# maxjiang216/corintho-ai

Measured on AMD Instinct MI355X. Metric: self-play games/sec at 400 sims/move, higher is better.
Workload: dtype f32(f16x3)

## Files before the change

### corintho_ai_amd/csrc/nn_rescnn.hip

```cpp
#include <hip/hip_runtime.h>
#include <math.h>
#include <stdlib.h>
#include <string.h>

#include <vector>

#include "engine_defs.h"
#include <memory>

#include "host.h"
#include "lds_dma.h"
#include "nn_split.h"

#define RC_NB 4
#define RC_POS_PER_WG 16
#define RC_STEM_CHUNK 1024
#define RC_CONV_CHUNK 4096
#define RC_NUM_CONVS 9
#define RC_NUM_CHUNKS 81
#define RC_TRUNK_FLOATS (9 * RC_STEM_CHUNK + 72 * RC_CONV_CHUNK)

typedef float f32x4 __attribute__((ext_vector_type(4)));

struct RcParams {
  const float *in;
  const int32_t *d_rows;
  const float *wtrunk;
  const float *epi;
  const float *whead;
  const float *head_epi;
  const float *wpol;
  const float *bpol;
  const float *wv1;
  const float *bv1;
  const float *wv2;
  const float *bv2;
  float *eval;
  float *probs;
  CoNetIO io;
};

__device__ __forceinline__ size_t rc_in_row(const RcParams &P, int pos) { return (size_t)(P.io.in_idx ? P.io.in_idx[pos] : pos); }
__device__ __forceinline__ size_t rc_out_row(const RcParams &P, int pos) { return (size_t)(P.io.out_idx ? P.io.out_idx[pos] : pos); }

__device__ __forceinline__ const float *rc_chunk_ptr(const float *wtrunk, int ch) {
  return ch < 9 ? wtrunk + ch * RC_STEM_CHUNK : wtrunk + 9 * RC_STEM_CHUNK + (ch - 9) * RC_CONV_CHUNK;
}

__device__ __forceinline__ void rc_stage(const float *wtrunk, float *lds_buf, int ch, int wave, int lane) {
  const float *src = rc_chunk_ptr(wtrunk, ch);
  const int pieces = ch < 9 ? RC_STEM_CHUNK / 256 : RC_CONV_CHUNK / 256;
  for (int p = wave; p < pieces; p += 4) {
    __builtin_amdgcn_global_load_lds((const void __attribute__((address_space(1))) *)(src + p * 256 + lane * 4),
                                     (void __attribute__((address_space(3))) *)(lds_buf + p * 256), 16, 0, 0);
  }
}

template <int S>
__device__ __forceinline__ float rc_row_shift(float v) {
  if (S == 0) return v;
  constexpr int ctrl = S > 0 ? (0x100 + S) : (0x110 - S);
  return __int_as_float(__builtin_amdgcn_mov_dpp(__float_as_int(v), ctrl, 0xF, 0xF, true));
}

template <int TAP>
__device__ __forceinline__ float rc_tap(float v, bool okL, bool okR) {
  constexpr int dy = TAP / 3 - 1, dx = TAP % 3 - 1;
  float s = rc_row_shift<4 * dy + dx>(v);
  if (dx == -1) s = okL ? s : 0.0f;
  if (dx == 1) s = okR ? s : 0.0f;
  return s;
}

template <int CT, int TAP>
__device__ __forceinline__ void rc_conv_tap(f32x4 (&acc)[RC_NB][4], const float (&in)[RC_NB][4][4], const float *w, int lane,
                                            bool okL, bool okR) {
#pragma unroll
  for (int t = 0; t < CT; ++t) {
#pragma unroll
    for (int r = 0; r < 4; ++r) {
      const float *wp = w + ((t * 4 + r) * 4) * 64 + lane;
      float a[4];
#pragma unroll
      for (int to = 0; to < 4; ++to) a[to] = wp[to * 64];
#pragma unroll
      for (int nb = 0; nb < RC_NB; ++nb) {
        const float b = rc_tap<TAP>(in[nb][t][r], okL, okR);
#pragma unroll
        for (int to = 0; to < 4; ++to) acc[nb][to] = __builtin_amdgcn_mfma_f32_16x16x4f32(a[to], b, acc[nb][to], 0, 0, 0);
      }
    }
  }
}

template <int CT>
__device__ __forceinline__ void rc_conv3x3(f32x4 (&acc)[RC_NB][4], const float (&in)[RC_NB][4][4], int &ch,
                                           const float *wtrunk, float *lds_w, int wave, int lane, bool okL, bool okR) {
#pragma unroll
  for (int nb = 0; nb < RC_NB; ++nb)
#pragma unroll
    for (int to = 0; to < 4; ++to) acc[nb][to] = (f32x4){0.f, 0.f, 0.f, 0.f};
#define RC_TAP(T)                                                                         \
  {                                                                                       \
    asm volatile("s_waitcnt vmcnt(0)" ::: "memory");                                      \
    __syncthreads();                                                                      \
    if (ch + 1 < RC_NUM_CHUNKS) rc_stage(wtrunk, lds_w + ((ch + 1) & 1) * RC_CONV_CHUNK, ch + 1, wave, lane); \
    rc_conv_tap<CT, T>(acc, in, lds_w + (ch & 1) * RC_CONV_CHUNK, lane, okL, okR);        \
    ++ch;                                                                                 \
  }
  RC_TAP(0) RC_TAP(1) RC_TAP(2) RC_TAP(3) RC_TAP(4) RC_TAP(5) RC_TAP(6) RC_TAP(7) RC_TAP(8)
#undef RC_TAP
}

template <bool ADD_SKIP, bool RELU>
__device__ __forceinline__ void rc_epilogue(float (&out)[RC_NB][4][4], const f32x4 (&acc)[RC_NB][4],
                                            const float (&skip)[RC_NB][4][4], const float *epi, int q) {
#pragma unroll
  for (int to = 0; to < 4; ++to) {
    const float4 b4 = *reinterpret_cast<const float4 *>(epi + 16 * to + 4 * q);
    const float4 a4 = *reinterpret_cast<const float4 *>(epi + 64 + 16 * to + 4 * q);
    const float4 c4 = *reinterpret_cast<const float4 *>(epi + 128 + 16 * to + 4 * q);
    const float bb[4] = {b4.x, b4.y, b4.z, b4.w};
    const float aa[4] = {a4.x, a4.y, a4.z, a4.w};
    const float cc[4] = {c4.x, c4.y, c4.z, c4.w};
#pragma unroll
    for (int nb = 0; nb < RC_NB; ++nb)
#pragma unroll
      for (int r = 0; r < 4; ++r) {
        float v = acc[nb][to][r] + bb[r];
        v = aa[r] * v + cc[r];
        if (ADD_SKIP) v = skip[nb][to][r] + v;
        if (RELU) v = v > 0.0f ? v : 0.0f;
        out[nb][to][r] = v;
      }
  }
}

__device__ __forceinline__ void rc_dense_policy(const RcParams &P, const float *wpol, const float *feat16, int rows,
                                                int pos_base, int lane, int ncols = 16);
__device__ __forceinline__ void rc_dense_value(const RcParams &P, const float *wv1, const float *wv2, const float *feat16,
                                               int rows, int pos_base, int lane, int ncols = 16);

__device__ __forceinline__ void rc_heads(const RcParams &P, const float (&x)[RC_NB][4][4], float *feat_wg, int wave,
                                         int rows, int row0, int lane, int q, int c) {
  float *feat_w = feat_wg + wave * RC_NB * 96;
  f32x4 h1[RC_NB];
#pragma unroll
  for (int nb = 0; nb < RC_NB; ++nb) h1[nb] = (f32x4){0.f, 0.f, 0.f, 0.f};
#pragma unroll
  for (int t = 0; t < 4; ++t)
#pragma unroll
    for (int r = 0; r < 4; ++r) {
      const float a = P.whead[(t * 4 + r) * 64 + lane];
#pragma unroll
      for (int nb = 0; nb < RC_NB; ++nb) h1[nb] = __builtin_amdgcn_mfma_f32_16x16x4f32(a, x[nb][t][r], h1[nb], 0, 0, 0);
    }
  {
    const float4 b4 = *reinterpret_cast<const float4 *>(P.head_epi + 4 * q);
    const float4 a4 = *reinterpret_cast<const float4 *>(P.head_epi + 16 + 4 * q);
    const float4 c4 = *reinterpret_cast<const float4 *>(P.head_epi + 32 + 4 * q);
    const float bb[4] = {b4.x, b4.y, b4.z, b4.w};
    const float aa[4] = {a4.x, a4.y, a4.z, a4.w};
    const float cc[4] = {c4.x, c4.y, c4.z, c4.w};
#pragma unroll
    for (int nb = 0; nb < RC_NB; ++nb)
#pragma unroll
      for (int r = 0; r < 4; ++r) {
        float v = h1[nb][r] + bb[r];
        v = aa[r] * v + cc[r];
        v = v > 0.0f ? v : 0.0f;
        if (q == 0) feat_w[nb * 96 + c * 4 + r] = v;
        if (q == 1 && r < 2) feat_w[nb * 96 + 64 + c * 2 + r] = v;
      }
  }
  __syncthreads();
  if (wave == 0) rc_dense_policy(P, P.wpol, feat_wg, rows, row0, lane);
  if (wave == 1) rc_dense_value(P, P.wv1, P.wv2, feat_wg, rows, row0, lane);
}

__device__ __forceinline__ void rc_dense_policy(const RcParams &P, const float *wpol, const float *feat16, int rows,
                                                int pos_base, int lane, int ncols) {
  const int q = lane >> 4, c = lane & 15;
  const float *feat = feat16 + c * 96;
  f32x4 pl[6];
#pragma unroll
  for (int to = 0; to < 6; ++to) pl[to] = (f32x4){0.f, 0.f, 0.f, 0.f};
#pragma unroll
  for (int s = 0; s < 16; ++s) {
    const float b = feat[4 * s + q];
#pragma unroll
    for (int to = 0; to < 6; ++to)
      pl[to] = __builtin_amdgcn_mfma_f32_16x16x4f32(wpol[(s * 6 + to) * 64 + lane], b, pl[to], 0, 0, 0);
  }
  float lg[6][4];
  float m = -INFINITY;
#pragma unroll
  for (int to = 0; to < 6; ++to) {
    const float4 b4 = *reinterpret_cast<const float4 *>(P.bpol + 16 * to + 4 * q);
    const float bb[4] = {b4.x, b4.y, b4.z, b4.w};
#pragma unroll
    for (int r = 0; r < 4; ++r) {
      lg[to][r] = pl[to][r] + bb[r];
      m = lg[to][r] > m ? lg[to][r] : m;
    }
  }
  float o = __shfl_xor(m, 16, 64);
  m = o > m ? o : m;
  o = __shfl_xor(m, 32, 64);
  m = o > m ? o : m;
  float sum = 0.0f;
#pragma unroll
  for (int to = 0; to < 6; ++to)
#pragma unroll
    for (int r = 0; r < 4; ++r) {
      lg[to][r] = __builtin_amdgcn_exp2f((lg[to][r] - m) * 1.44269504088896340736f);
      sum += lg[to][r];
    }
  sum += __shfl_xor(sum, 16, 64);
  sum += __shfl_xor(sum, 32, 64);
  const float inv = 1.0f / sum;
  const int pos = pos_base + c;
  if (pos < rows && c < ncols) {
    const size_t orow = rc_out_row(P, pos);
#pragma unroll
    for (int to = 0; to < 6; ++to) {
      float4 p = make_float4(lg[to][0] * inv, lg[to][1] * inv, lg[to][2] * inv, lg[to][3] * inv);
      *reinterpret_cast<float4 *>(P.probs + orow * (size_t)P.io.probs_stride + 16 * to + 4 * q) = p;
    }
  }
}

__device__ __forceinline__ void rc_dense_value(const RcParams &P, const float *wv1, const float *wv2, const float *feat16,
                                               int rows, int pos_base, int lane, int ncols) {
  const int q = lane >> 4, c = lane & 15;
  const float *feat = feat16 + c * 96;
  f32x4 v1[4];
#pragma unroll
  for (int to = 0; to < 4; ++to) v1[to] = (f32x4){0.f, 0.f, 0.f, 0.f};
#pragma unroll
  for (int s = 0; s < 8; ++s) {
    const float b = feat[64 + 4 * s + q];
#pragma unroll
    for (int to = 0; to < 4; ++to)
      v1[to] = __builtin_amdgcn_mfma_f32_16x16x4f32(wv1[(s * 4 + to) * 64 + lane], b, v1[to], 0, 0, 0);
  }
  f32x4 v2 = (f32x4){0.f, 0.f, 0.f, 0.f};
#pragma unroll
  for (int t = 0; t < 4; ++t) {
    const float4 b4 = *reinterpret_cast<const float4 *>(P.bv1 + 16 * t + 4 * q);
    const float bb[4] = {b4.x, b4.y, b4.z, b4.w};
#pragma unroll
    for (int r = 0; r < 4; ++r) {
      float hv = v1[t][r] + bb[r];
      hv = hv > 0.0f ? hv : 0.0f;
      v2 = __builtin_amdgcn_mfma_f32_16x16x4f32(wv2[(t * 4 + r) * 64 + lane], hv, v2, 0, 0, 0);
    }
  }
  const int pos = pos_base + c;
  if (q == 0 && pos < rows && c < ncols) P.eval[rc_out_row(P, pos) * (size_t)P.io.eval_stride] = tanhf(v2[0] + P.bv2[0]);
}

#define CO_RC_F32_BLOCKS 2
__global__ __launch_bounds__(256, CO_RC_F32_BLOCKS) void co_k_rescnn_forward(RcParams P) {
  __shared__ __attribute__((aligned(16))) float lds_w[2 * RC_CONV_CHUNK];
  __shared__ float lds_feat[4][RC_NB][96];
  const int rows = *P.d_rows;
  const int row0 = blockIdx.x * RC_POS_PER_WG;
  if (row0 >= rows) return;
  const int tid = threadIdx.x;
  const int wave = tid >> 6, lane = tid & 63, q = lane >> 4, c = lane & 15;
  const bool okL = (c & 3) != 0, okR = (c & 3) != 3;
  rc_stage(P.wtrunk, lds_w, 0, wave, lane);

  float x[RC_NB][4][4];
#pragma unroll
  for (int nb = 0; nb < RC_NB; ++nb) {
    const int pos = row0 + wave * RC_NB + nb;
    float4 v = make_float4(0.f, 0.f, 0.f, 0.f);
    if (pos < rows) v = *reinterpret_cast<const float4 *>(P.in + rc_in_row(P, pos) * CO_STATE_STRIDE + (q == 0 ? 4 * c : 60 + 4 * q));
#pragma unroll
    for (int t = 0; t < 4; ++t)
#pragma unroll
      for (int r = 0; r < 4; ++r) x[nb][t][r] = 0.0f;
    x[nb][0][0] = v.x;
    x[nb][0][1] = v.y;
    x[nb][0][2] = v.z;
    x[nb][0][3] = v.w;
  }

  f32x4 acc[RC_NB][4];
  float y[RC_NB][4][4];
  int ch = 0;
  rc_conv3x3<1>(acc, x, ch, P.wtrunk, lds_w, wave, lane, okL, okR);
  rc_epilogue<false, true>(x, acc, x, P.epi, q);
  for (int b = 0; b < 4; ++b) {
    rc_conv3x3<4>(acc, x, ch, P.wtrunk, lds_w, wave, lane, okL, okR);
    rc_epilogue<false, true>(y, acc, x, P.epi + (size_t)(1 + 2 * b) * 192, q);
    rc_conv3x3<4>(acc, y, ch, P.wtrunk, lds_w, wave, lane, okL, okR);
    rc_epilogue<true, true>(x, acc, x, P.epi + (size_t)(2 + 2 * b) * 192, q);
  }

  rc_heads(P, x, &lds_feat[0][0][0], wave, rows, row0, lane, q, c);
}

#include "nn_rescnn_split.h"
#include "nn_rescnn_pix.h"

struct ResCnnNet : CoNet {
  std::vector<DevBuf<float>> bufs;
  RcParams P;
  size_t cap;

  float *upload(const std::vector<float> &h, rt_stream_t s) {
    bufs.emplace_back();
    bufs.back().upload(h.data(), h.size(), s);
    return bufs.back().p;
  }

  ResCnnNet(const float *w, size_t max_rows, rt_stream_t s) : cap(max_rows) {
    constexpr ResCnnLayout RL;
    std::vector<float> trunk(RC_TRUNK_FLOATS, 0.0f), epi((size_t)RC_NUM_CONVS * 192, 0.0f);
    size_t off = 0;
    for (int cv = 0; cv < RC_NUM_CONVS; ++cv) {
      const int cin = RL.cin(cv), ct = cv == 0 ? 1 : 4;
      const size_t chunk = cv == 0 ? RC_STEM_CHUNK : RC_CONV_CHUNK;
      const float *K = w + RL.kernel(cv);
      for (int tap = 0; tap < 9; ++tap)
        for (int t = 0; t < ct; ++t)
          for (int r = 0; r < 4; ++r)
            for (int to = 0; to < 4; ++to)
              for (int q = 0; q < 4; ++q)
                for (int i = 0; i < 16; ++i) {
                  int ci = 16 * t + 4 * q + r, co = 16 * to + i;
                  float v = ci < cin ? K[((size_t)tap * cin + ci) * 64 + co] : 0.0f;
                  trunk[off + (size_t)tap * chunk + ((size_t)(t * 4 + r) * 4 + to) * 64 + 16 * q + i] = v;
                }
      off += 9 * chunk;
      for (int i = 0; i < 64; ++i) epi[(size_t)cv * 192 + i] = w[RL.bias(cv) + i];
      bn_fold(w, RL, cv, 64, &epi[(size_t)cv * 192 + 64], &epi[(size_t)cv * 192 + 128]);
    }
    const float *pk = w + RL.p_k, *pb = w + RL.bias(9), *pdk = w + RL.p_dk, *pdb = w + RL.p_db;
    const float *vk = w + RL.v_k, *vb = w + RL.bias(10);
    const float *vd1k = w + RL.v_d1k, *vd1b = w + RL.v_d1b, *vd2k = w + RL.v_d2k, *vd2b = w + RL.v_d2b;
    std::vector<float> whead(16 * 64, 0.0f), hepi(48, 0.0f), wpol(16 * 6 * 64, 0.0f), bpol(pdb, pdb + 96);
    std::vector<float> wv1(8 * 4 * 64, 0.0f), bv1(vd1b, vd1b + 64), wv2(16 * 64, 0.0f), bv2(vd2b, vd2b + 1);
    for (int t = 0; t < 4; ++t)
      for (int r = 0; r < 4; ++r)
        for (int q = 0; q < 4; ++q)
          for (int i = 0; i < 16; ++i) {
            int k = 16 * t + 4 * q + r;
            float v = i < 4 ? pk[k * 4 + i] : i < 6 ? vk[k * 2 + (i - 4)] : 0.0f;
            whead[(size_t)(t * 4 + r) * 64 + 16 * q + i] = v;
            wv2[(size_t)(t * 4 + r) * 64 + 16 * q + i] = i == 0 ? vd2k[k] : 0.0f;
          }
    for (int i = 0; i < 4; ++i) hepi[i] = pb[i];
    for (int i = 0; i < 2; ++i) hepi[4 + i] = vb[i];
    bn_fold(w, RL, 9, 4, &hepi[16], &hepi[32]);
    bn_fold(w, RL, 10, 2, &hepi[16 + 4], &hepi[32 + 4]);
    for (int s2 = 0; s2 < 16; ++s2)
      for (int to = 0; to < 6; ++to)
        for (int q = 0; q < 4; ++q)
          for (int i = 0; i < 16; ++i) wpol[((size_t)s2 * 6 + to) * 64 + 16 * q + i] = pdk[(size_t)(4 * s2 + q) * 96 + 16 * to + i];
    for (int s2 = 0; s2 < 8; ++s2)
      for (int to = 0; to < 4; ++to)
        for (int q = 0; q < 4; ++q)
          for (int i = 0; i < 16; ++i) wv1[((size_t)s2 * 4 + to) * 64 + 16 * q + i] = vd1k[(size_t)(4 * s2 + q) * 64 + 16 * to + i];
    memset(&P, 0, sizeof P);
    P.wtrunk = upload(trunk, s);
    P.epi = upload(epi, s);
    P.whead = upload(whead, s);
    P.head_epi = upload(hepi, s);
    P.wpol = upload(wpol, s);
    P.bpol = upload(bpol, s);
    P.wv1 = upload(wv1, s);
    P.bv1 = upload(bv1, s);
    P.wv2 = upload(wv2, s);
    P.bv2 = upload(bv2, s);
    rt_sync(s);
  }
  size_t max_rows() const override { return cap; }
  int kind() const override { return co_net_kind_of(CO_FAMILY_RESCNN4, 0, false); }
  double flop_per_row() const override { return ResCnnLayout().flop_per_row(); }
  void forward(const float *d_in, int32_t rows_cap, const int32_t *d_rows, float *d_eval, float *d_probs,
               rt_stream_t s, const CoNetIO &io = CoNetIO()) override {
    int grid = (rows_cap + RC_POS_PER_WG - 1) / RC_POS_PER_WG;
    if (grid < 1) return;
    RT_LAUNCH(co_k_rescnn_forward, grid, 256, s, launch_params(d_in, d_rows, d_eval, d_probs, io));
  }
  RcParams launch_params(const float *d_in, const int32_t *d_rows, float *d_eval, float *d_probs, const CoNetIO &io) const {
    RcParams p = P;
    p.io = io, p.in = d_in, p.d_rows = d_rows, p.eval = d_eval, p.probs = d_probs;
    return p;
  }
};

struct ResCnnSplitNet : ResCnnNet {
  int nt;
  bool f16;
  int num_cus = 256;
  DevBuf<uint32_t> d_trunk3, d_whead3, d_epi3;
  RangeFlag range;
  ResCnnSplitNet(const float *w, size_t max_rows, rt_stream_t s, int nterms, bool fp16 = false)
      : ResCnnNet(w, max_rows, s), nt(nterms), f16(fp16) {
    const std::vector<uint32_t> tr = co_pack_rescnn_trunk(w, nt, f16), wh3 = co_pack_rescnn_head(w, nt, f16);
    const size_t frag1 = wh3.size(), head_words = RCS_HEAD_WORDS(nt);
    d_trunk3.upload(tr.data(), tr.size(), s);
    d_whead3.alloc(head_words, s);
    rt_h2d(d_whead3.p, wh3.data(), wh3.size() * 4, s);
    rt_d2d(d_whead3.p + frag1, P.wpol, 6144 * 4, s);
    rt_d2d(d_whead3.p + frag1 + 6144, P.wv1, 2048 * 4, s);
    rt_d2d(d_whead3.p + frag1 + 6144 + 2048, P.wv2, 1024 * 4, s);
    if (f16) range.alloc(s);
    d_epi3.alloc(RC3_EPI_WORDS, s);
    rt_d2d(d_epi3.p, P.epi, (size_t)RC_NUM_CONVS * 192 * 4, s);
    if (nt == 2) {
      rt_max_dynamic_lds(co_k_rescnn_forward_x3, RCS_LDS_WORDS(2, 2) * 4);
      rt_max_dynamic_lds(co_k_rescnn_forward_x3_small, RCS_LDS_WORDS(2, 1) * 4);
      rt_max_dynamic_lds(co_k_rescnn_forward_h3p, RCP_LDS_WORDS * 4);
      rt_max_dynamic_lds(co_k_rescnn_forward_h3_small, RCS_LDS_WORDS(2, 1) * 4);
      int dev = 0;
      hipDeviceProp_t prop;
      if (hipGetDevice(&dev) == hipSuccess && hipGetDeviceProperties(&prop, dev) == hipSuccess && prop.multiProcessorCount > 0)
        num_cus = prop.multiProcessorCount;
    } else {
      rt_max_dynamic_lds(co_k_rescnn_forward_x6, RCS_LDS_WORDS(3, 1) * 4);
    }
    rt_sync(s);
  }
  bool range_exceeded(rt_stream_t s) override { return range.read(s); }
  int kind() const override { return co_net_kind_of(CO_FAMILY_RESCNN4, nt, f16); }
  void forward(const float *d_in, int32_t rows_cap, const int32_t *d_rows, float *d_eval, float *d_probs,
               rt_stream_t s, const CoNetIO &io = CoNetIO()) override {
    if (rows_cap < 1) return;
    Rc3Params q;
    q.base = launch_params(d_in, d_rows, d_eval, d_probs, io);
    q.wtrunk = d_trunk3.p;
    q.whead3 = d_whead3.p;
    q.epi3 = d_epi3.p;
    q.range_flag = range.ptr();
    q.pass_rows = f16 && io.alone ? 32 * num_cus : 0;
    if (nt == 2) {
      const int small_rows = rows_cap < RC3_SMALL_ROWS ? rows_cap : RC3_SMALL_ROWS;
      const int thin_rows = rows_cap < RC6_THIN_ROWS ? rows_cap : RC6_THIN_ROWS;
      const int small_grid = f16 && (thin_rows + 7) / 8 > (small_rows + 15) / 16 ? (thin_rows + 7) / 8 : (small_rows + 15) / 16;
      RT_LAUNCH_LDS(f16 ? co_k_rescnn_forward_h3_small : co_k_rescnn_forward_x3_small, small_grid, 512, RCS_LDS_WORDS(2, 1) * 4, s, q);
      if (rows_cap > RC3_SMALL_ROWS) {
        if (f16)
          RT_LAUNCH_LDS(co_k_rescnn_forward_h3p, (rows_cap + 31) / 32, 512, RCP_LDS_WORDS * 4, s, q);
        else
          RT_LAUNCH_LDS(co_k_rescnn_forward_x3, (rows_cap + 31) / 32, 512, RCS_LDS_WORDS(2, 2) * 4, s, q);
      }
    } else {
      const int thin_rows = rows_cap < RC6_THIN_ROWS ? rows_cap : RC6_THIN_ROWS;
      const int grid = (rows_cap + 15) / 16 > (thin_rows + 7) / 8 ? (rows_cap + 15) / 16 : (thin_rows + 7) / 8;
      RT_LAUNCH_LDS(co_k_rescnn_forward_x6, grid, 512, RCS_LDS_WORDS(3, 1) * 4, s, q);
    }
  }
};

struct ResCnnH3NetGroup : CoNetGroup {
  DevBuf<uint32_t> d_w;
  RangeFlag range;
  size_t cap;
  int m;
  uint32_t stride = 0, off_epi = 0, off_head = 0, off_small = 0;
  ResCnnH3NetGroup(const float *const *w, int models, size_t max_rows, rt_stream_t s) : cap(max_rows), m(models) {
    for (int i = 0; i < models; ++i) {
      std::unique_ptr<ResCnnSplitNet> one;
      try {
        one.reset(new ResCnnSplitNet(w[i], max_rows, s, 2, true));
      } catch (const std::invalid_argument &e) {
        throw std::invalid_argument("model " + std::to_string(i) + " of the group: " + e.what());
      }
      if (i == 0) {
        off_epi = (uint32_t)one->d_trunk3.n;
        off_head = off_epi + RC3_EPI_WORDS;
        off_small = off_head + RCS_HEAD_WORDS(2);
        stride = off_small + RCG_SMALL_WORDS;
        d_w.alloc((size_t)models * stride, s);
      }
      uint32_t *dst = d_w.p + (size_t)i * stride;
      rt_d2d(dst, one->d_trunk3.p, (size_t)off_epi * 4, s);
      rt_d2d(dst + off_epi, one->d_epi3.p, (size_t)RC3_EPI_WORDS * 4, s);
      rt_d2d(dst + off_head, one->d_whead3.p, (size_t)RCS_HEAD_WORDS(2) * 4, s);
      rt_d2d(dst + off_small, one->P.head_epi, 48 * 4, s);
      rt_d2d(dst + off_small + 48, one->P.bpol, 96 * 4, s);
      rt_d2d(dst + off_small + 144, one->P.bv1, 64 * 4, s);
      rt_d2d(dst + off_small + 208, one->P.bv2, 4, s);
      rt_sync(s);
    }
    range.alloc(s);
    rt_sync(s);
    rt_max_dynamic_lds(co_k_rescnn_forward_h3_grouped, RCS_LDS_WORDS(2, 1) * 4);
  }
  int kind() const override { return co_net_kind_of(CO_FAMILY_RESCNN4, 2, true); }
  int models() const override { return m; }
  size_t max_rows() const override { return cap; }
  bool grouped_kernel() const override { return true; }
  int tile() const override { return RCG_POS_PER_WG; }
  bool range_exceeded(rt_stream_t s) override { return range.read(s); }
  void forward(const float *d_in, int32_t rows_cap, const CoGroupPlan &plan, float *d_eval, float *d_probs, rt_stream_t s) override {
    int grid = rows_cap / RCG_POS_PER_WG + m;
    if (grid > plan.wg_cap) grid = plan.wg_cap;
    if (grid < 1 || plan.seg_stride) return;
    RcGroupParams g;
    g.in = d_in, g.wg = plan.wg, g.n_wg = plan.n_wg, g.idx = plan.idx, g.wbase = d_w.p;
    g.stride = stride, g.off_epi = off_epi, g.off_head = off_head, g.off_small = off_small;
    g.eval = d_eval, g.probs = d_probs, g.range_flag = range.ptr();
    RT_LAUNCH_LDS(co_k_rescnn_forward_h3_grouped, grid, 512, RCS_LDS_WORDS(2, 1) * 4, s, g);
  }
};

CoNetGroup *co_rescnn_h3_group_create(const float *const *weights, int models, size_t n_floats, size_t max_rows, rt_stream_t s) {
  if (n_floats != (size_t)CO_RESCNN4_NUM_WEIGHTS) return nullptr;
  return new ResCnnH3NetGroup(weights, models, max_rows, s);
}

CoNet *co_rescnn_create(const float *weights, size_t n_floats, size_t max_rows, rt_stream_t s) {
  if (n_floats != (size_t)CO_RESCNN4_NUM_WEIGHTS) return nullptr;
  return new ResCnnNet(weights, max_rows, s);
}

CoNet *co_rescnn_split_create(const float *weights, size_t n_floats, size_t max_rows, rt_stream_t s, int nterms, bool f16) {
  if (n_floats != (size_t)CO_RESCNN4_NUM_WEIGHTS || (nterms != 2 && nterms != 3) || (f16 && nterms != 2)) return nullptr;
  return new ResCnnSplitNet(weights, max_rows, s, nterms, f16);
}
```

### corintho_ai_amd/csrc/nn_rescnn_split.h

```cpp
#pragma once
#define RC3_SMALL_ROWS 4096
#define RC6_THIN_ROWS 2048
#define RC3_EPI_WORDS 1792
#define RCS_DENSE_WORDS (6144 + 2048 + 1024)
#define RCS_HEAD_WORDS(NT) (RCS_FRAG1_WORDS(NT) + RCS_DENSE_WORDS)
#define RC3_NUM_GROUPS 27
#define RCS_GROUP_WORDS(NT) (3 * RCS_CONV_CHUNK(NT))
#define RCS_FEAT_WORDS(NP) (8 * 2 * (NP) * 96)
#define RCS_LDS_WORDS(NT, NP) \
  (2 * RCS_GROUP_WORDS(NT) + ((NT) == 2 ? RCS_FEAT_WORDS(NP) : 0) + RC3_EPI_WORDS + ((NT) == 2 ? RCS_HEAD_WORDS(NT) : 0))

struct Rc3Params {
  RcParams base;
  const uint32_t *wtrunk;
  const uint32_t *whead3;
  const uint32_t *epi3;
  uint32_t *range_flag;
  int32_t pass_rows;
};

__device__ __forceinline__ int rcp_small_begin(const Rc3Params &Q, int rows) {
  if (rows <= RC3_SMALL_ROWS) return 0;
  if (Q.pass_rows <= 0) return rows;
  const int full = rows / Q.pass_rows * Q.pass_rows;
  return rows - full > RC3_SMALL_ROWS ? rows : full;
}

template <int NT>
__device__ __forceinline__ const uint32_t *rcs_group_ptr(const uint32_t *wtrunk, int gi) {
  return gi < 3 ? wtrunk + gi * 3 * RCS_STEM_CHUNK(NT) : wtrunk + 9 * RCS_STEM_CHUNK(NT) + (gi - 3) * 3 * RCS_CONV_CHUNK(NT);
}

__device__ __forceinline__ void rcs_stage_words(const uint32_t *src, uint32_t lds_addr, int words, int wave, int lane,
                                                int nw = 8) {
  const int pieces = words / 256;
  for (int p = wave; p < pieces; p += nw) co_lds_dma_1k(src + p * 256 + lane * 4, lds_addr + (uint32_t)p * 1024u);
}

template <int NT>
__device__ __forceinline__ void rcs_stage(const uint32_t *wtrunk, uint32_t lds_addr, int gi, int wave, int lane, int nw = 8) {
  rcs_stage_words(rcs_group_ptr<NT>(wtrunk, gi), lds_addr, gi < 3 ? 3 * RCS_STEM_CHUNK(NT) : 3 * RCS_CONV_CHUNK(NT), wave, lane, nw);
}

template <int S>
__device__ __forceinline__ uint32_t rc3_row_shift(uint32_t v) {
  if (S == 0) return v;
  constexpr int ctrl = S > 0 ? (0x100 + S) : (0x110 - S);
  return (uint32_t)__builtin_amdgcn_mov_dpp((int)v, ctrl, 0xF, 0xF, true);
}

#define RC3_CNDMASK_DPP4(CTRL)                                                                          \
  asm("s_mov_b64 vcc, %[m]\n\t"                                                                         \
      "v_cndmask_b32_dpp %[o0], %[i0], %[z], vcc " CTRL " row_mask:0xf bank_mask:0xf bound_ctrl:1\n\t"   \
      "v_cndmask_b32_dpp %[o1], %[i1], %[z], vcc " CTRL " row_mask:0xf bank_mask:0xf bound_ctrl:1\n\t"   \
      "v_cndmask_b32_dpp %[o2], %[i2], %[z], vcc " CTRL " row_mask:0xf bank_mask:0xf bound_ctrl:1\n\t"   \
      "v_cndmask_b32_dpp %[o3], %[i3], %[z], vcc " CTRL " row_mask:0xf bank_mask:0xf bound_ctrl:1\n\t"   \
      "s_nop 1"                                                                                         \
      : [o0] "=&v"(o0), [o1] "=&v"(o1), [o2] "=&v"(o2), [o3] "=&v"(o3)                                  \
      : [i0] "v"(in[0]), [i1] "v"(in[1]), [i2] "v"(in[2]), [i3] "v"(in[3]), [z] "v"(zero), [m] "s"(wrap) \
      : "vcc")

template <int TAP>
__device__ __forceinline__ u32x4 rc3_tap4(const uint32_t (&in)[4], uint32_t zero) {
  constexpr int dy = TAP / 3 - 1, dx = TAP % 3 - 1;
  u32x4 out;
  if constexpr (dx == 0) {
#pragma unroll
    for (int m = 0; m < 4; ++m) out[m] = rc3_row_shift<4 * dy>(in[m]);
  } else {
    const unsigned long long wrap = dx < 0 ? 0x1111111111111111ull : 0x8888888888888888ull;
    uint32_t o0, o1, o2, o3;
    if constexpr (4 * dy + dx == -5) RC3_CNDMASK_DPP4("row_shr:5");
    if constexpr (4 * dy + dx == -3) RC3_CNDMASK_DPP4("row_shr:3");
    if constexpr (4 * dy + dx == -1) RC3_CNDMASK_DPP4("row_shr:1");
    if constexpr (4 * dy + dx == 1) RC3_CNDMASK_DPP4("row_shl:1");
    if constexpr (4 * dy + dx == 3) RC3_CNDMASK_DPP4("row_shl:3");
    if constexpr (4 * dy + dx == 5) RC3_CNDMASK_DPP4("row_shl:5");
    out[0] = o0;
    out[1] = o1;
    out[2] = o2;
    out[3] = o3;
  }
  return out;
}

__device__ __forceinline__ u32x4 rc3_tap4_sel(const uint32_t (&in)[4], int tap, uint32_t zero) {
  switch (tap) {
    case 0: return rc3_tap4<0>(in, zero);
    case 1: return rc3_tap4<1>(in, zero);
    case 2: return rc3_tap4<2>(in, zero);
    case 3: return rc3_tap4<3>(in, zero);
    case 4: return rc3_tap4<4>(in, zero);
    case 5: return rc3_tap4<5>(in, zero);
    case 6: return rc3_tap4<6>(in, zero);
    case 7: return rc3_tap4<7>(in, zero);
    default: return rc3_tap4<8>(in, zero);
  }
}

template <int CS, int G, int NP, int NT, bool F16 = false>
__device__ __forceinline__ void rcs_conv_group(f32x16 (&acc)[NP][2], const uint32_t (&p)[NT][NP][4][4], const uint32_t *wg,
                                               int lane) {
  constexpr int XT = CS == 1 ? 1 : NT;
  constexpr int tw = CS == 1 ? RCS_STEM_CHUNK(NT) : RCS_CONV_CHUNK(NT);
  constexpr int N = 3 * CS;
  uint32_t zero;
  asm("v_mov_b32 %0, 0" : "=v"(zero));
  u32x4 a[2][NT][2];
#pragma unroll
  for (int to = 0; to < 2; ++to)
#pragma unroll
    for (int t = 0; t < NT; ++t) a[0][t][to] = *reinterpret_cast<const u32x4 *>(wg + (((0 * 2 + to) * NT + t) * 64 + lane) * 4);
#pragma unroll
  for (int idx = 0; idx < N; ++idx) {
    const int cur = idx & 1, nxt = cur ^ 1;
    const int tg = idx / CS, s = idx % CS;
    if (idx + 1 < N) {
      const int tg1 = (idx + 1) / CS, s1 = (idx + 1) % CS;
      const uint32_t *w1 = wg + tg1 * tw;
#pragma unroll
      for (int to = 0; to < 2; ++to)
#pragma unroll
        for (int t = 0; t < NT; ++t)
          a[nxt][t][to] = *reinterpret_cast<const u32x4 *>(w1 + (((s1 * 2 + to) * NT + t) * 64 + lane) * 4);
    }
#pragma unroll
    for (int np = 0; np < NP; ++np) {
      u32x4 B[XT];
#pragma unroll
      for (int t = 0; t < XT; ++t) B[t] = rc3_tap4_sel(p[t][np][s], 3 * G + tg, zero);
#pragma unroll
      for (int sum = 0; sum < NT; ++sum)
#pragma unroll
        for (int i = 0; i <= sum; ++i)
          if (sum - i < XT) {
#pragma unroll
            for (int to = 0; to < 2; ++to)
              co_mfma_32x32x16<F16>(acc[np][to], a[cur][i][to], B[sum - i]);
          }
    }
  }
}

template <int CS, int NP, int NT, int NW, bool F16 = false>
__device__ __forceinline__ void rcs_conv3x3(f32x16 (&acc)[NP][2], const uint32_t (&p)[NT][NP][4][4], int &ch,
                                            const Rc3Params &Q, uint32_t *lds_w, uint32_t lds_w_addr, int wave, int lane) {
#pragma unroll
  for (int np = 0; np < NP; ++np)
#pragma unroll
    for (int to = 0; to < 2; ++to)
#pragma unroll
      for (int i = 0; i < 16; ++i) acc[np][to][i] = 0.0f;
#define RC3_GROUP(G)                                                                                              \
  {                                                                                                               \
    CO_WAIT_VMCNT(0);                                          \
    co_wg_barrier();                              \
    if (ch + 1 < RC3_NUM_GROUPS)                                                                                  \
      rcs_stage<NT>(Q.wtrunk, lds_w_addr + (uint32_t)((ch + 1) & 1) * (RCS_GROUP_WORDS(NT) * 4u), ch + 1, wave, lane, NW); \
    else if (NT != 2)                         \
      rcs_stage_words(Q.whead3, lds_w_addr + (uint32_t)((ch + 1) & 1) * (RCS_GROUP_WORDS(NT) * 4u), RCS_HEAD_WORDS(NT), wave, lane, NW); \
    rcs_conv_group<CS, G, NP, NT, F16>(acc, p, lds_w + (ch & 1) * RCS_GROUP_WORDS(NT), lane);                          \
    ++ch;                                                                                                         \
  }
  RC3_GROUP(0) RC3_GROUP(1) RC3_GROUP(2)
#undef RC3_GROUP
}

template <int NP, int NT, bool F16 = false>
__device__ __forceinline__ void rcs_pack(uint32_t (&p)[NT][NP][4][4], const float (&v)[NP][2][16], uint32_t &amax) {
#pragma unroll
  for (int np = 0; np < NP; ++np)
#pragma unroll
    for (int T = 0; T < 2; ++T)
#pragma unroll
      for (int a = 0; a < 2; ++a)
#pragma unroll
        for (int m = 0; m < 4; ++m) {
          uint32_t t[NT];
          co_split_pair<NT, F16>(v[np][T][8 * a + 2 * m], v[np][T][8 * a + 2 * m + 1], t);
          if constexpr (F16) amax = co_pk_max_f16(amax, t[0]);
#pragma unroll
          for (int i = 0; i < NT; ++i) p[i][np][2 * T + a][m] = t[i];
        }
}

template <bool ADD_SKIP, int NP>
__device__ __forceinline__ void rc3_epilogue(float (&out)[NP][2][16], const f32x16 (&acc)[NP][2],
                                             const float (&skip)[NP][2][16], const float *epi, int h) {
#pragma unroll
  for (int T = 0; T < 2; ++T)
#pragma unroll
    for (int g = 0; g < 4; ++g) {
      const int chn = 32 * T + 8 * g + 4 * h;
      const float4 b4 = *reinterpret_cast<const float4 *>(epi + chn);
      const float4 a4 = *reinterpret_cast<const float4 *>(epi + 64 + chn);
      const float4 c4 = *reinterpret_cast<const float4 *>(epi + 128 + chn);
      const float bb[4] = {b4.x, b4.y, b4.z, b4.w};
      const float aa[4] = {a4.x, a4.y, a4.z, a4.w};
      const float cc[4] = {c4.x, c4.y, c4.z, c4.w};
      float cb[4];
#pragma unroll
      for (int i = 0; i < 4; ++i) cb[i] = __builtin_fmaf(aa[i], bb[i], cc[i]);
#pragma unroll
      for (int np = 0; np < NP; ++np)
#pragma unroll
        for (int i = 0; i < 4; ++i) {
          float v = __builtin_fmaf(aa[i], acc[np][T][4 * g + i], cb[i]);
          if (ADD_SKIP) v = skip[np][T][4 * g + i] + v;
          v = v > 0.0f ? v : 0.0f;
          out[np][T][4 * g + i] = v;
        }
    }
}

#ifdef CO_PROF
__device__ unsigned long long rc3_prof[12];
#define RC3_STAMP(slot)                                                              \
  {                                                                                  \
    unsigned long long now_ = __builtin_readcyclecounter();                          \
    if (tid == 0) atomicAdd(&rc3_prof[slot], now_ - stamp_);                         \
    stamp_ = now_;                                                                   \
  }
extern "C" int ca_net_prof(unsigned long long out[12]) {
  return hipMemcpyFromSymbol(out, HIP_SYMBOL(rc3_prof), sizeof(rc3_prof)) == hipSuccess ? 0 : 1;
}
__device__ unsigned rc3_trace[8 * 20];
extern "C" int ca_net_trace(unsigned out[160]) {
  return hipMemcpyFromSymbol(out, HIP_SYMBOL(rc3_trace), sizeof(rc3_trace)) == hipSuccess ? 0 : 1;
}
#else
#define RC3_STAMP(slot)
#endif

template <int NP, int NT, int NW = 8, bool F16 = false, bool GROUPED = false>
__device__ __forceinline__ void rcs_forward(const Rc3Params &Q, const int rbase = 0, const int g_end = 0) {
  const RcParams &P = Q.base;
  extern __shared__ __attribute__((aligned(16))) uint32_t lds_dyn[];
  uint32_t *lds_w = lds_dyn;
  float *lds_feat = reinterpret_cast<float *>(NT == 2 ? lds_dyn + 2 * RCS_GROUP_WORDS(NT) : lds_dyn);
  const int rows = GROUPED ? g_end : *P.d_rows;
  if (!GROUPED && NT == 2 && (rows - rbase <= RC3_SMALL_ROWS) != (NP == 1)) return;
  const int row0 = GROUPED ? rbase : rbase + (int)blockIdx.x * (2 * NP * NW);
  if (row0 >= rows) return;
  const int tid = threadIdx.x;
  const int wave = __builtin_amdgcn_readfirstlane(tid >> 6), lane = tid & 63, h = lane >> 5, p2 = (lane >> 4) & 1, c = lane & 15;
#ifdef CO_PROF
  unsigned long long stamp_ = __builtin_readcyclecounter();
  const unsigned long long start_ = stamp_, real_ = __builtin_amdgcn_s_memrealtime();
#endif
  const uint32_t lds_w_addr = co_lds_addr(lds_dyn);
  constexpr int epi_off = 2 * RCS_GROUP_WORDS(NT) + (NT == 2 ? RCS_FEAT_WORDS(NP) : 0);
  uint32_t *lds_epi_w = lds_dyn + epi_off;
  const uint32_t lds_epi_addr = lds_w_addr + epi_off * 4u;
  const uint32_t *lds_head = NT == 2 ? lds_epi_w + RC3_EPI_WORDS : lds_w + (RC3_NUM_GROUPS & 1) * RCS_GROUP_WORDS(NT);

  float x[NP][2][16];
#pragma unroll
  for (int np = 0; np < NP; ++np) {
    const int pos = row0 + wave * (2 * NP) + np * 2 + p2;
#pragma unroll
    for (int T = 0; T < 2; ++T)
#pragma unroll
      for (int i = 0; i < 16; ++i) x[np][T][i] = 0.0f;
    if (pos < rows) {
      const float *row = P.in + rc_in_row(P, pos) * CO_STATE_STRIDE;
      const float4 v0 = *reinterpret_cast<const float4 *>(row + (h == 0 ? 4 * c : 64));
      const float4 v1 = *reinterpret_cast<const float4 *>(row + (h == 0 ? 68 : 72));
      x[np][0][0] = v0.x; x[np][0][1] = v0.y; x[np][0][2] = v0.z; x[np][0][3] = v0.w;
      x[np][0][4] = v1.x; x[np][0][5] = v1.y; x[np][0][6] = v1.z; x[np][0][7] = v1.w;
    }
  }
  uint32_t pk[NT][NP][4][4];
  uint32_t amax = 0u;
  rcs_pack<NP, NT, F16>(pk, x, amax);
  rcs_stage<NT>(Q.wtrunk, lds_w_addr, 0, wave, lane, NW);
  rcs_stage_words(Q.epi3, lds_epi_addr, RC3_EPI_WORDS, wave, lane, NW);
  if (NT == 2) rcs_stage_words(Q.whead3, lds_epi_addr + RC3_EPI_WORDS * 4u, RCS_HEAD_WORDS(NT), wave, lane, NW);
  RC3_STAMP(0)
  f32x16 acc[NP][2];
  float y[NP][2][16];
  int ch = 0;
  rcs_conv3x3<1, NP, NT, NW, F16>(acc, pk, ch, Q, lds_w, lds_w_addr, wave, lane);
  RC3_STAMP(1)
  const float *lds_epi = reinterpret_cast<const float *>(lds_epi_w);
  rc3_epilogue<false, NP>(x, acc, x, lds_epi, h);
  rcs_pack<NP, NT, F16>(pk, x, amax);
  RC3_STAMP(2)
  for (int b = 0; b < 4; ++b) {
    rcs_conv3x3<4, NP, NT, NW, F16>(acc, pk, ch, Q, lds_w, lds_w_addr, wave, lane);
    RC3_STAMP(3)
    rc3_epilogue<false, NP>(y, acc, x, lds_epi + (1 + 2 * b) * 192, h);
    rcs_pack<NP, NT, F16>(pk, y, amax);
    RC3_STAMP(2)
    rcs_conv3x3<4, NP, NT, NW, F16>(acc, pk, ch, Q, lds_w, lds_w_addr, wave, lane);
    RC3_STAMP(3)
    rc3_epilogue<true, NP>(x, acc, x, lds_epi + (2 + 2 * b) * 192, h);
    rcs_pack<NP, NT, F16>(pk, x, amax);
    RC3_STAMP(2)
  }
  if constexpr (F16) co_raise_unless_f16_finite(amax, Q.range_flag);
  if (NT != 2) {
    CO_WAIT_VMCNT(0);
    co_wg_barrier();
  }
  float *feat_w = lds_feat + wave * (2 * NP) * 96;
  u32x4 hw[NT][4];
#pragma unroll
  for (int s = 0; s < 4; ++s)
#pragma unroll
    for (int t = 0; t < NT; ++t) hw[t][s] = *reinterpret_cast<const u32x4 *>(lds_head + ((s * NT + t) * 64 + lane) * 4);
#pragma unroll
  for (int np = 0; np < NP; ++np) {
    f32x16 h1;
#pragma unroll
    for (int i = 0; i < 16; ++i) h1[i] = 0.0f;
#pragma unroll
    for (int s = 0; s < 4; ++s) {
      u32x4 B[NT];
#pragma unroll
      for (int t = 0; t < NT; ++t) {
#pragma unroll
        for (int m = 0; m < 4; ++m) B[t][m] = pk[t][np][s][m];
      }
#pragma unroll
      for (int sum = 0; sum < NT; ++sum)
#pragma unroll
        for (int i = 0; i <= sum; ++i) co_mfma_32x32x16<F16>(h1, hw[i][s], B[sum - i]);
    }
    const float4 b4 = *reinterpret_cast<const float4 *>(P.head_epi + 4 * h);
    const float4 a4 = *reinterpret_cast<const float4 *>(P.head_epi + 16 + 4 * h);
    const float4 c4 = *reinterpret_cast<const float4 *>(P.head_epi + 32 + 4 * h);
    const float bb[4] = {b4.x, b4.y, b4.z, b4.w};
    const float aa[4] = {a4.x, a4.y, a4.z, a4.w};
    const float cc[4] = {c4.x, c4.y, c4.z, c4.w};
    const int pw = np * 2 + p2;
#pragma unroll
    for (int r = 0; r < 4; ++r) {
      float v = h1[r] + bb[r];
      v = aa[r] * v + cc[r];
      v = v > 0.0f ? v : 0.0f;
      if (h == 0) feat_w[pw * 96 + c * 4 + r] = v;
      if (h == 1 && r < 2) feat_w[pw * 96 + 64 + c * 2 + r] = v;
    }
  }
  RC3_STAMP(4)
  __syncthreads();
  const float *lds_dense = reinterpret_cast<const float *>(lds_head + RCS_FRAG1_WORDS(NT));
  constexpr int wgpos = 2 * NP * NW, ntiles = (wgpos + 15) / 16;
  constexpr int ncols = wgpos < 16 ? wgpos : 16;
  if (wave < ntiles)
    rc_dense_policy(P, lds_dense, lds_feat + wave * 16 * 96, rows, row0 + wave * 16, lane, ncols);
  else if (wave >= 2 && wave < 2 + ntiles)
    rc_dense_value(P, lds_dense + 6144, lds_dense + 6144 + 2048, lds_feat + (wave - 2) * 16 * 96, rows,
                   row0 + (wave - 2) * 16, lane, ncols);
  RC3_STAMP(5)
#ifdef CO_PROF
  if (tid == 0) {
    atomicAdd(&rc3_prof[6], __builtin_readcyclecounter() - start_);
    atomicAdd(&rc3_prof[7], 1ull);
    atomicAdd(&rc3_prof[8], __builtin_amdgcn_s_memrealtime() - real_);
  }
#endif
}

__global__ __launch_bounds__(512, 2) void co_k_rescnn_forward_x3(Rc3Params Q) { rcs_forward<2, 2>(Q); }
__global__ __launch_bounds__(512, 2) void co_k_rescnn_forward_x3_small(Rc3Params Q) { rcs_forward<1, 2>(Q); }
__global__ __launch_bounds__(512, 2) void co_k_rescnn_forward_x6(Rc3Params Q) {
  if (*Q.base.d_rows <= RC6_THIN_ROWS) {
    if (threadIdx.x >= 256) return;
    rcs_forward<1, 3, 4>(Q);
  } else {
    rcs_forward<1, 3, 8>(Q);
  }
}

__global__ __launch_bounds__(512, 2) void co_k_rescnn_forward_h3_small(Rc3Params Q) {
  const int rows = *Q.base.d_rows, rbase = rcp_small_begin(Q, rows);
  if (rows - rbase <= 0) return;
  if (rows - rbase <= RC6_THIN_ROWS) {
    if (threadIdx.x >= 256) return;
    rcs_forward<1, 2, 4, true>(Q, rbase);
  } else {
    rcs_forward<1, 2, 8, true>(Q, rbase);
  }
}


#define RCG_POS_PER_WG 16
#define RCG_SMALL_WORDS 256
struct RcGroupParams {
  const float *in;
  const CoGroupWG *wg;
  const int32_t *n_wg, *idx;
  const uint32_t *wbase;
  uint32_t stride, off_epi, off_head, off_small;
  float *eval, *probs;
  uint32_t *range_flag;
};
__global__ __launch_bounds__(512, 2) void co_k_rescnn_forward_h3_grouped(RcGroupParams G) {
  if ((int)blockIdx.x >= *G.n_wg) return;
  const CoGroupWG e = G.wg[blockIdx.x];
  const int first = __builtin_amdgcn_readfirstlane(e.first), count = __builtin_amdgcn_readfirstlane(e.count);
  const uint32_t *w = G.wbase + (size_t)__builtin_amdgcn_readfirstlane(e.model) * G.stride;
  const float *small = reinterpret_cast<const float *>(w + G.off_small);
  Rc3Params Q;
  Q.base.in = G.in, Q.base.d_rows = nullptr;
  Q.base.wtrunk = nullptr, Q.base.epi = nullptr, Q.base.whead = nullptr, Q.base.wpol = nullptr, Q.base.wv1 = nullptr, Q.base.wv2 = nullptr;
  Q.base.head_epi = small, Q.base.bpol = small + 48, Q.base.bv1 = small + 144, Q.base.bv2 = small + 208;
  Q.base.eval = G.eval, Q.base.probs = G.probs;
  Q.base.io = CoNetIO();
  Q.base.io.in_idx = Q.base.io.out_idx = G.idx;
  Q.wtrunk = w, Q.epi3 = w + G.off_epi, Q.whead3 = w + G.off_head;
  Q.range_flag = G.range_flag, Q.pass_rows = 0;
  rcs_forward<1, 2, 8, true, true>(Q, first, first + count);
}
```

Before: 10730.

## Add dedicated thin-batch f16 ResCNN kernel with 4-slot weight pipeline

Adds a new 256-thread kernel for small f16 batches (up to the thin-row threshold). Each wave handles two positions and weights stream through a four-slot LDS ring, so two items stay in flight behind the one being consumed. The forward path now launches this kernel first and only launches the small and large kernels for larger batches. This is meant to cut per-workgroup LDS and latency for small self-play batches, at the cost of an extra kernel launch and more code to maintain.

```diff
diff --git a/corintho_ai_amd/csrc/nn_rescnn.hip b/corintho_ai_amd/csrc/nn_rescnn.hip
--- a/corintho_ai_amd/csrc/nn_rescnn.hip
+++ b/corintho_ai_amd/csrc/nn_rescnn.hip
@@ -418,6 +418,7 @@
       rt_max_dynamic_lds(co_k_rescnn_forward_x3_small, RCS_LDS_WORDS(2, 1) * 4);
       rt_max_dynamic_lds(co_k_rescnn_forward_h3p, RCP_LDS_WORDS * 4);
       rt_max_dynamic_lds(co_k_rescnn_forward_h3_small, RCS_LDS_WORDS(2, 1) * 4);
+      rt_max_dynamic_lds(co_k_rescnn_forward_h3_thin, RCT_LDS_WORDS * 4);
       int dev = 0;
       hipDeviceProp_t prop;
       if (hipGetDevice(&dev) == hipSuccess && hipGetDeviceProperties(&prop, dev) == hipSuccess && prop.multiProcessorCount > 0)
@@ -439,17 +440,18 @@
     q.epi3 = d_epi3.p;
     q.range_flag = range.ptr();
     q.pass_rows = f16 && io.alone ? 32 * num_cus : 0;
-    if (nt == 2) {
+    if (nt == 2 && f16) {
+      const int thin_rows = rows_cap < RC6_THIN_ROWS ? rows_cap : RC6_THIN_ROWS;
+      RT_LAUNCH_LDS(co_k_rescnn_forward_h3_thin, (thin_rows + RCT_POS_PER_WG - 1) / RCT_POS_PER_WG, 64 * RCT_WAVES, RCT_LDS_WORDS * 4, s, q);
+      if (rows_cap > RC6_THIN_ROWS) {
+        const int small_rows = rows_cap < RC3_SMALL_ROWS ? rows_cap : RC3_SMALL_ROWS;
+        RT_LAUNCH_LDS(co_k_rescnn_forward_h3_small, (small_rows + 15) / 16, 512, RCS_LDS_WORDS(2, 1) * 4, s, q);
+      }
+      if (rows_cap > RC3_SMALL_ROWS) RT_LAUNCH_LDS(co_k_rescnn_forward_h3p, (rows_cap + 31) / 32, 512, RCP_LDS_WORDS * 4, s, q);
+    } else if (nt == 2) {
       const int small_rows = rows_cap < RC3_SMALL_ROWS ? rows_cap : RC3_SMALL_ROWS;
-      const int thin_rows = rows_cap < RC6_THIN_ROWS ? rows_cap : RC6_THIN_ROWS;
-      const int small_grid = f16 && (thin_rows + 7) / 8 > (small_rows + 15) / 16 ? (thin_rows + 7) / 8 : (small_rows + 15) / 16;
-      RT_LAUNCH_LDS(f16 ? co_k_rescnn_forward_h3_small : co_k_rescnn_forward_x3_small, small_grid, 512, RCS_LDS_WORDS(2, 1) * 4, s, q);
-      if (rows_cap > RC3_SMALL_ROWS) {
-        if (f16)
-          RT_LAUNCH_LDS(co_k_rescnn_forward_h3p, (rows_cap + 31) / 32, 512, RCP_LDS_WORDS * 4, s, q);
-        else
-          RT_LAUNCH_LDS(co_k_rescnn_forward_x3, (rows_cap + 31) / 32, 512, RCS_LDS_WORDS(2, 2) * 4, s, q);
-      }
+      RT_LAUNCH_LDS(co_k_rescnn_forward_x3_small, (small_rows + 15) / 16, 512, RCS_LDS_WORDS(2, 1) * 4, s, q);
+      if (rows_cap > RC3_SMALL_ROWS) RT_LAUNCH_LDS(co_k_rescnn_forward_x3, (rows_cap + 31) / 32, 512, RCS_LDS_WORDS(2, 2) * 4, s, q);
     } else {
       const int thin_rows = rows_cap < RC6_THIN_ROWS ? rows_cap : RC6_THIN_ROWS;
       const int grid = (rows_cap + 15) / 16 > (thin_rows + 7) / 8 ? (rows_cap + 15) / 16 : (thin_rows + 7) / 8;
diff --git a/corintho_ai_amd/csrc/nn_rescnn_split.h b/corintho_ai_amd/csrc/nn_rescnn_split.h
--- a/corintho_ai_amd/csrc/nn_rescnn_split.h
+++ b/corintho_ai_amd/csrc/nn_rescnn_split.h
@@ -376,13 +376,217 @@
 
 __global__ __launch_bounds__(512, 2) void co_k_rescnn_forward_h3_small(Rc3Params Q) {
   const int rows = *Q.base.d_rows, rbase = rcp_small_begin(Q, rows);
-  if (rows - rbase <= 0) return;
-  if (rows - rbase <= RC6_THIN_ROWS) {
-    if (threadIdx.x >= 256) return;
-    rcs_forward<1, 2, 4, true>(Q, rbase);
-  } else {
-    rcs_forward<1, 2, 8, true>(Q, rbase);
-  }
+  if (rows - rbase <= RC6_THIN_ROWS) return;
+  rcs_forward<1, 2, 8, true>(Q, rbase);
+}
+
+#define RCT_SLOTS 4
+#define RCT_NUM_ITEMS 82
+#define RCT_WAVES 4
+#define RCT_POS_PER_WG (2 * RCT_WAVES)
+#define RCT_FEAT_WORDS (RCT_POS_PER_WG * 96)
+#define RCT_LDS_WORDS (RCT_SLOTS * RCS_CONV_CHUNK(2) + RCT_FEAT_WORDS + RC3_EPI_WORDS)
+static_assert(RCT_LDS_WORDS * 4 <= 81920, "two workgroups of the thin kernel share a compute unit's 160 KB of LDS");
+static_assert(RCT_FEAT_WORDS + RC3_EPI_WORDS >= 16 * 96, "the dense heads' feature reads stay inside the workgroup's LDS");
+
+__device__ __forceinline__ int rct_pieces(int g) { return g < 9 ? 1 : g < 81 ? 4 : g < RCT_NUM_ITEMS ? 2 : 0; }
+static_assert(RCS_STEM_CHUNK(2) == 1 * RCT_WAVES * 256 && RCS_CONV_CHUNK(2) == 4 * RCT_WAVES * 256 &&
+                  RCS_FRAG1_WORDS(2) == 2 * RCT_WAVES * 256,
+              "rct_pieces: every wave issues the same number of transfers for an item");
+
+template <int N>
+__device__ __forceinline__ void rct_stage_pieces(const uint32_t *src, uint32_t lds_addr, int wave, int lane) {
+#pragma unroll
+  for (int k = 0; k < N; ++k) {
+    const int p = wave + k * RCT_WAVES;
+    co_lds_dma_1k(src + p * 256 + lane * 4, lds_addr + (uint32_t)p * 1024u);
+  }
+}
+
+__device__ __forceinline__ void rct_stage(const Rc3Params &Q, uint32_t lds_w_addr, int g, int wave, int lane) {
+  if (g >= RCT_NUM_ITEMS) return;
+  const uint32_t dst = lds_w_addr + (uint32_t)(g % RCT_SLOTS) * (RCS_CONV_CHUNK(2) * 4u);
+  if (g < 9) rct_stage_pieces<1>(Q.wtrunk + g * RCS_STEM_CHUNK(2), dst, wave, lane);
+  else if (g < 81) rct_stage_pieces<4>(Q.wtrunk + 9 * RCS_STEM_CHUNK(2) + (g - 9) * RCS_CONV_CHUNK(2), dst, wave, lane);
+  else rct_stage_pieces<2>(Q.whead3, dst, wave, lane);
+}
+
+__device__ __forceinline__ void rct_wait(int g) {
+  static_assert(RCT_SLOTS == 4, "rct_wait counts two items in flight behind the one waited for");
+  switch (rct_pieces(g + 1) + rct_pieces(g + 2)) {
+    case 8: CO_WAIT_VMCNT(8); break;
+    case 6: CO_WAIT_VMCNT(6); break;
+    case 5: CO_WAIT_VMCNT(5); break;
+    case 2: CO_WAIT_VMCNT(2); break;
+    default: CO_WAIT_VMCNT(0); break;
+  }
+}
+
+template <int CS>
+__device__ __forceinline__ void rct_conv_tap(f32x16 (&acc)[1][2], const uint32_t (&p)[2][1][4][4], const uint32_t *wt, int tap, int lane) {
+  constexpr int XT = CS == 1 ? 1 : 2;
+  uint32_t zero;
+  asm("v_mov_b32 %0, 0" : "=v"(zero));
+  u32x4 a[2][2][2];
+#pragma unroll
+  for (int to = 0; to < 2; ++to)
+#pragma unroll
+    for (int t = 0; t < 2; ++t) a[0][t][to] = *reinterpret_cast<const u32x4 *>(wt + (((0 * 2 + to) * 2 + t) * 64 + lane) * 4);
+#pragma unroll
+  for (int s = 0; s < CS; ++s) {
+    const int cur = s & 1, nxt = cur ^ 1;
+    if (s + 1 < CS) {
+#pragma unroll
+      for (int to = 0; to < 2; ++to)
+#pragma unroll
+        for (int t = 0; t < 2; ++t)
+          a[nxt][t][to] = *reinterpret_cast<const u32x4 *>(wt + ((((s + 1) * 2 + to) * 2 + t) * 64 + lane) * 4);
+    }
+    u32x4 B[XT];
+#pragma unroll
+    for (int t = 0; t < XT; ++t) B[t] = rc3_tap4_sel(p[t][0][s], tap, zero);
+#pragma unroll
+    for (int sum = 0; sum < 2; ++sum)
+#pragma unroll
+      for (int i = 0; i <= sum; ++i)
+        if (sum - i < XT) {
+#pragma unroll
+          for (int to = 0; to < 2; ++to) co_mfma_32x32x16<true>(acc[0][to], a[cur][i][to], B[sum - i]);
+        }
+  }
+}
+
+template <int CS>
+__device__ __forceinline__ void rct_conv3x3(f32x16 (&acc)[1][2], const uint32_t (&p)[2][1][4][4], int &g, const Rc3Params &Q,
+                                            const uint32_t *lds_w, uint32_t lds_w_addr, int wave, int lane) {
+#pragma unroll
+  for (int to = 0; to < 2; ++to)
+#pragma unroll
+    for (int i = 0; i < 16; ++i) acc[0][to][i] = 0.0f;
+#pragma unroll
+  for (int tap = 0; tap < 9; ++tap, ++g) {
+    rct_wait(g);
+    co_wg_barrier();
+    rct_stage(Q, lds_w_addr, g + RCT_SLOTS - 1, wave, lane);
+    rct_conv_tap<CS>(acc, p, lds_w + (g % RCT_SLOTS) * RCS_CONV_CHUNK(2), tap, lane);
+  }
+}
+
+__global__ __launch_bounds__(256, 2) void co_k_rescnn_forward_h3_thin(Rc3Params Q) {
+  const RcParams &P = Q.base;
+  extern __shared__ __attribute__((aligned(16))) uint32_t lds_dyn[];
+  const int rows = *P.d_rows, rbase = rcp_small_begin(Q, rows);
+  if (rows - rbase > RC6_THIN_ROWS) return;
+  const int row0 = rbase + (int)blockIdx.x * RCT_POS_PER_WG;
+  if (row0 >= rows) return;
+  const int tid = threadIdx.x;
+  const int wave = __builtin_amdgcn_readfirstlane(tid >> 6), lane = tid & 63, h = lane >> 5, p2 = (lane >> 4) & 1, c = lane & 15;
+#ifdef CO_PROF
+  unsigned long long stamp_ = __builtin_readcyclecounter();
+  const unsigned long long start_ = stamp_, real_ = __builtin_amdgcn_s_memrealtime();
+#endif
+  const uint32_t *lds_w = lds_dyn;
+  const uint32_t lds_w_addr = co_lds_addr(lds_dyn);
+  float *lds_feat = reinterpret_cast<float *>(lds_dyn + RCT_SLOTS * RCS_CONV_CHUNK(2));
+  constexpr int epi_off = RCT_SLOTS * RCS_CONV_CHUNK(2) + RCT_FEAT_WORDS;
+  const float *lds_epi = reinterpret_cast<const float *>(lds_dyn + epi_off);
+
+  float x[1][2][16];
+  {
+    const int pos = row0 + wave * 2 + p2;
+#pragma unroll
+    for (int T = 0; T < 2; ++T)
+#pragma unroll
+      for (int i = 0; i < 16; ++i) x[0][T][i] = 0.0f;
+    if (pos < rows) {
+      const float *row = P.in + rc_in_row(P, pos) * CO_STATE_STRIDE;
+      const float4 v0 = *reinterpret_cast<const float4 *>(row + (h == 0 ? 4 * c : 64));
+      const float4 v1 = *reinterpret_cast<const float4 *>(row + (h == 0 ? 68 : 72));
+      x[0][0][0] = v0.x; x[0][0][1] = v0.y; x[0][0][2] = v0.z; x[0][0][3] = v0.w;
+      x[0][0][4] = v1.x; x[0][0][5] = v1.y; x[0][0][6] = v1.z; x[0][0][7] = v1.w;
+    }
+  }
+  uint32_t pk[2][1][4][4];
+  uint32_t amax = 0u;
+  rcs_pack<1, 2, true>(pk, x, amax);
+  rcs_stage_words(Q.epi3, lds_w_addr + epi_off * 4u, RC3_EPI_WORDS, wave, lane, RCT_WAVES);
+#pragma unroll
+  for (int g0 = 0; g0 < RCT_SLOTS - 1; ++g0) rct_stage(Q, lds_w_addr, g0, wave, lane);
+  RC3_STAMP(0)
+  f32x16 acc[1][2];
+  float y[1][2][16];
+  int g = 0;
+  rct_conv3x3<1>(acc, pk, g, Q, lds_w, lds_w_addr, wave, lane);
+  RC3_STAMP(1)
+  rc3_epilogue<false, 1>(x, acc, x, lds_epi, h);
+  rcs_pack<1, 2, true>(pk, x, amax);
+  RC3_STAMP(2)
+  for (int b = 0; b < 4; ++b) {
+    rct_conv3x3<4>(acc, pk, g, Q, lds_w, lds_w_addr, wave, lane);
+    RC3_STAMP(3)
+    rc3_epilogue<false, 1>(y, acc, x, lds_epi + (1 + 2 * b) * 192, h);
+    rcs_pack<1, 2, true>(pk, y, amax);
+    RC3_STAMP(2)
+    rct_conv3x3<4>(acc, pk, g, Q, lds_w, lds_w_addr, wave, lane);
+    RC3_STAMP(3)
+    rc3_epilogue<true, 1>(x, acc, x, lds_epi + (2 + 2 * b) * 192, h);
+    rcs_pack<1, 2, true>(pk, x, amax);
+    RC3_STAMP(2)
+  }
+  co_raise_unless_f16_finite(amax, Q.range_flag);
+  CO_WAIT_VMCNT(0);
+  co_wg_barrier();
+  {
+    const uint32_t *lds_head = lds_w + ((RCT_NUM_ITEMS - 1) % RCT_SLOTS) * RCS_CONV_CHUNK(2);
+    float *feat_w = lds_feat + wave * 2 * 96;
+    u32x4 hw[2][4];
+#pragma unroll
+    for (int s = 0; s < 4; ++s)
+#pragma unroll
+      for (int t = 0; t < 2; ++t) hw[t][s] = *reinterpret_cast<const u32x4 *>(lds_head + ((s * 2 + t) * 64 + lane) * 4);
+    f32x16 h1;
+#pragma unroll
+    for (int i = 0; i < 16; ++i) h1[i] = 0.0f;
+#pragma unroll
+    for (int s = 0; s < 4; ++s) {
+      u32x4 B[2];
+#pragma unroll
+      for (int t = 0; t < 2; ++t) {
+#pragma unroll
+        for (int m = 0; m < 4; ++m) B[t][m] = pk[t][0][s][m];
+      }
+#pragma unroll
+      for (int sum = 0; sum < 2; ++sum)
+#pragma unroll
+        for (int i = 0; i <= sum; ++i) co_mfma_32x32x16<true>(h1, hw[i][s], B[sum - i]);
+    }
+    const float4 b4 = *reinterpret_cast<const float4 *>(P.head_epi + 4 * h);
+    const float4 a4 = *reinterpret_cast<const float4 *>(P.head_epi + 16 + 4 * h);
+    const float4 c4 = *reinterpret_cast<const float4 *>(P.head_epi + 32 + 4 * h);
+    const float bb[4] = {b4.x, b4.y, b4.z, b4.w};
+    const float aa[4] = {a4.x, a4.y, a4.z, a4.w};
+    const float cc[4] = {c4.x, c4.y, c4.z, c4.w};
+#pragma unroll
+    for (int r = 0; r < 4; ++r) {
+      float v = h1[r] + bb[r];
+      v = aa[r] * v + cc[r];
+      v = v > 0.0f ? v : 0.0f;
+      if (h == 0) feat_w[p2 * 96 + c * 4 + r] = v;
+      if (h == 1 && r < 2) feat_w[p2 * 96 + 64 + c * 2 + r] = v;
+    }
+  }
+  RC3_STAMP(4)
+  __syncthreads();
+  if (wave == 0) rc_dense_policy(P, P.wpol, lds_feat, rows, row0, lane, RCT_POS_PER_WG);
+  else if (wave == 2) rc_dense_value(P, P.wv1, P.wv2, lds_feat, rows, row0, lane, RCT_POS_PER_WG);
+  RC3_STAMP(5)
+#ifdef CO_PROF
+  if (tid == 0) {
+    atomicAdd(&rc3_prof[6], __builtin_readcyclecounter() - start_);
+    atomicAdd(&rc3_prof[7], 1ull);
+    atomicAdd(&rc3_prof[8], __builtin_amdgcn_s_memrealtime() - real_);
+  }
+#endif
 }
 
 
```

After: 10750 (median of 6 runs). About the same (+0.2%).
